# meyer-lab/cmtf-pls

Measured on AMD Instinct MI355X. Metric: nipals_iters_per_sec, higher is better.
Workload: dtype f32

## Files before the change

### cmtf_pls_amd/csrc/mixed.hip

```cpp
#include "common.hpp"

namespace cmtfpls {

typedef float f4_t __attribute__((ext_vector_type(4)));

#ifndef CMTFPLS_MIXED_UN
#define CMTFPLS_MIXED_UN 4
#endif
#ifndef CMTFPLS_MIXED_FAST
#define CMTFPLS_MIXED_FAST 1
#endif
#ifndef CMTFPLS_MIXED_UN_WIDE
#define CMTFPLS_MIXED_UN_WIDE 4
#endif

void launch_reduce_rows(const double* part, int nrows, int64_t P, double* out, hipStream_t st);

template <bool MASKED, bool VEC, int MT, bool FAST>
__global__ __launch_bounds__(256) void xcov_mixed_kernel(const float* __restrict__ X, int64_t I, int64_t P,
                                                        const double* __restrict__ Y, int ldy, int M,
                                                        double* __restrict__ part, int rows_per_block) {
  const int lane = threadIdx.x & 63, wv = threadIdx.x >> 6;
  const int kq = lane >> 4, nn = lane & 15;
  const int64_t cb = ((int64_t)blockIdx.x * 4 + wv) * 64;
  if (cb >= P) return;
  const int64_t c = cb + 4 * nn;
  const int64_t r0 = (int64_t)blockIdx.y * rows_per_block;
  const int64_t r1 = (r0 + rows_per_block < I) ? r0 + rows_per_block : I;
  using XV = Pack<float, 4>;
  f4_t acc32[MT][4];
  double acc64[MT][4][4];
#pragma unroll
  for (int mt = 0; mt < MT; ++mt)
#pragma unroll
    for (int e = 0; e < 4; ++e) {
      acc32[mt][e] = f4_t{0.f, 0.f, 0.f, 0.f};
#pragma unroll
      for (int g = 0; g < 4; ++g) acc64[mt][e][g] = 0.0;
    }
  bool mok[MT];
  int ycol[MT];
#pragma unroll
  for (int mt = 0; mt < MT; ++mt) { mok[mt] = (mt * 16 + nn) < M; ycol[mt] = mok[mt] ? mt * 16 + nn : M - 1; }
  constexpr int UN = (MT >= 2) ? CMTFPLS_MIXED_UN_WIDE : CMTFPLS_MIXED_UN;
  constexpr int FLUSH_TRIPS = 64 / (8 * UN);
  const int64_t cc = (c < P) ? c : (VEC ? P - 4 : P - 1);

  auto load_stage = [&](XV (&x)[UN], double (&a)[UN][MT], int64_t r) {
#pragma unroll
    for (int s = 0; s < UN; ++s) {
      const int64_t row = r + 4 * s + kq;
      const int64_t rowc = (FAST || row < r1) ? row : r1 - 1;
      if (VEC) {
        x[s] = ld_stream(reinterpret_cast<const XV*>(X + rowc * P + cc));
      } else {
#pragma unroll
        for (int e = 0; e < 4; ++e) x[s].e[e] = X[rowc * P + ((cc + e < P) ? cc + e : P - 1)];
      }
#pragma unroll
      for (int mt = 0; mt < MT; ++mt) a[s][mt] = Y[rowc * ldy + ycol[mt]];
    }
  };
  auto mma_stage = [&](const XV (&x)[UN], const double (&a)[UN][MT], int64_t r) {
#pragma unroll
    for (int s = 0; s < UN; ++s) {
      const bool rok = FAST || (r + 4 * s + kq) < r1;
      float af[MT];
#pragma unroll
      for (int mt = 0; mt < MT; ++mt) af[mt] = (FAST || (rok && mok[mt])) ? (float)a[s][mt] : 0.f;
#pragma unroll
      for (int e = 0; e < 4; ++e) {
        float xv = x[s].e[e];
        if (MASKED) xv = (xv == xv) ? xv : 0.f;
        const float b = (FAST || (rok && c + e < P)) ? xv : 0.f;
#pragma unroll
        for (int mt = 0; mt < MT; ++mt)
          acc32[mt][e] = __builtin_amdgcn_mfma_f32_16x16x4f32(af[mt], b, acc32[mt][e], 0, 0, 0);
      }
    }
  };
  auto flush = [&]() {
#pragma unroll
    for (int mt = 0; mt < MT; ++mt)
#pragma unroll
      for (int e = 0; e < 4; ++e) {
#pragma unroll
        for (int g = 0; g < 4; ++g) acc64[mt][e][g] += (double)acc32[mt][e][g];
        acc32[mt][e] = f4_t{0.f, 0.f, 0.f, 0.f};
      }
  };

  XV xa[UN], xb[UN];
  double aa[UN][MT], ab[UN][MT];
  load_stage(xa, aa, r0);
  int trip = 0;
  for (int64_t r = r0; r < r1; r += 8 * UN, ++trip) {
    load_stage(xb, ab, r + 4 * UN);
    __builtin_amdgcn_sched_barrier(0);
    mma_stage(xa, aa, r);
    __builtin_amdgcn_sched_barrier(0);
    load_stage(xa, aa, (FAST && r + 8 * UN >= r1) ? r : r + 8 * UN);
    __builtin_amdgcn_sched_barrier(0);
    mma_stage(xb, ab, r + 4 * UN);
    __builtin_amdgcn_sched_barrier(0);
    if (trip % FLUSH_TRIPS == FLUSH_TRIPS - 1) flush();
  }
  flush();
#pragma unroll
  for (int mt = 0; mt < MT; ++mt)
#pragma unroll
    for (int g = 0; g < 4; ++g) {
      const int m = mt * 16 + kq * 4 + g;
      if (m < M) {
        double* dst = part + ((int64_t)blockIdx.y * M + m) * P + c;
#pragma unroll
        for (int e = 0; e < 4; ++e)
          if (c + e < P) dst[e] = acc64[mt][e][g];
      }
    }
}

template <bool VEC, int RT>
__global__ __launch_bounds__(256) void mttkrp_mixed_kernel(const float* __restrict__ X, int64_t I, int A, int B,
                                                          const double* __restrict__ WA, const double* __restrict__ WB, int R,
                                                          double* __restrict__ out, int ldo) {
  extern __shared__ double lds[];
  constexpr int RP = 16 * RT;
  double* sA = lds;
  double* sB = lds + (size_t)A * RP;
  for (int idx = threadIdx.x; idx < A * RP; idx += 256) { const int j = idx / RP, r = idx % RP; sA[idx] = (r < R) ? WA[(int64_t)j * R + r] : 0.0; }
  for (int idx = threadIdx.x; idx < B * RP; idx += 256) { const int k = idx / RP, r = idx % RP; sB[idx] = (r < R) ? WB[(int64_t)k * R + r] : 0.0; }
  __syncthreads();
  const int lane = threadIdx.x & 63, wv = threadIdx.x >> 6;
  const int ri = lane & 15, kq = lane >> 4;
  const int64_t P = (int64_t)A * B;
  const int64_t ngroups = (I + 15) / 16;
  using XV = Pack<float, 4>;
  for (int64_t grp = (int64_t)blockIdx.x * 4 + wv; grp < ngroups; grp += (int64_t)gridDim.x * 4) {
    const int64_t i0 = grp * 16;
    const bool rok = (i0 + ri) < I;
    const float* __restrict__ xr = X + (rok ? i0 + ri : I - 1) * P;
    f4_t acc32[RT];
    double acc64[RT][4];
#pragma unroll
    for (int t = 0; t < RT; ++t) {
      acc32[t] = f4_t{0.f, 0.f, 0.f, 0.f};
#pragma unroll
      for (int g = 0; g < 4; ++g) acc64[t][g] = 0.0;
    }
    KronWalk w(4 * kq, 16, B);
    constexpr int UN = 4;
    int trip = 0;
    for (int64_t c0 = 0; c0 < P; c0 += 16 * UN, ++trip) {
      XV x[UN];
#pragma unroll
      for (int s = 0; s < UN; ++s) {
        const int64_t c = c0 + 16 * s + 4 * kq;
        if (VEC) {
          x[s] = ld_stream(reinterpret_cast<const XV*>(xr + ((c < P) ? c : P - 4)));
        } else {
#pragma unroll
          for (int e = 0; e < 4; ++e) x[s].e[e] = xr[(c + e < P) ? c + e : P - 1];
        }
      }
#pragma unroll
      for (int s = 0; s < UN; ++s) {
        const int64_t c = c0 + 16 * s + 4 * kq;
#pragma unroll
        for (int e = 0; e < 4; ++e) {
          const bool ok = rok && (c + e < P);
          const float a = ok ? x[s].e[e] : 0.f;
          int j = w.j, k = w.k + e;
          if (!VEC && k >= B) { j += k / B; k = k % B; }
          const bool wok = (c + e < P);
#pragma unroll
          for (int t = 0; t < RT; ++t) {
            const float b = wok ? (float)(sA[(size_t)j * RP + t * 16 + ri] * sB[(size_t)k * RP + t * 16 + ri]) : 0.f;
            acc32[t] = __builtin_amdgcn_mfma_f32_16x16x4f32(a, b, acc32[t], 0, 0, 0);
          }
        }
        w.next();
      }
      if ((trip & 3) == 3) {
#pragma unroll
        for (int t = 0; t < RT; ++t) {
#pragma unroll
          for (int g = 0; g < 4; ++g) acc64[t][g] += (double)acc32[t][g];
          acc32[t] = f4_t{0.f, 0.f, 0.f, 0.f};
        }
      }
    }
#pragma unroll
    for (int t = 0; t < RT; ++t)
#pragma unroll
      for (int g = 0; g < 4; ++g) {
        const int64_t row = i0 + kq * 4 + g;
        const int r = t * 16 + ri;
        if (row < I && r < R) out[row * ldo + r] = acc64[t][g] + (double)acc32[t][g];
      }
  }
}

template <int NL>
__global__ __launch_bounds__(256) void mttkrp_kj_mixed_kernel(const float* __restrict__ X, int64_t I, int A, int B,
                                                              const double* __restrict__ WA, const double* __restrict__ WB, int R,
                                                              double* __restrict__ out, int ldo) {
  constexpr int V = 4, RP = 16, CHJ = 8 / NL, KP = NL * 16 * V;
  constexpr int FLUSH = 64 / CHJ;
  extern __shared__ double lds[];
  double* sB = lds;
  float* sA = reinterpret_cast<float*>(lds + (size_t)B * RP);
  for (int idx = threadIdx.x; idx < A * RP; idx += 256) { const int j = idx / RP, r = idx % RP; sA[idx] = (r < R) ? (float)WA[(int64_t)j * R + r] : 0.f; }
  for (int idx = threadIdx.x; idx < B * RP; idx += 256) { const int k = idx / RP, r = idx % RP; sB[idx] = (r < R) ? WB[(int64_t)k * R + r] : 0.0; }
  __syncthreads();
  const int lane = threadIdx.x & 63, wv = threadIdx.x >> 6;
  const int kk = lane & 15, jq = lane >> 4;
  const int64_t P = (int64_t)A * B;
  const int npass = B / KP, cpp = A / (4 * CHJ);
  const int nchunks = npass * cpp, npairs = nchunks / 2;
  const int64_t istep = (int64_t)gridDim.x * 4;
  using XV = Pack<float, V>;
  XV b0[CHJ][NL], b1[CHJ][NL];
  auto load = [&](XV (&buf)[CHJ][NL], const float* __restrict__ xs, int q) {
    const int ps = q / cpp, c = q - ps * cpp;
    const float* __restrict__ xp = xs + (int64_t)(c * CHJ * 4) * B + ps * KP;
#pragma unroll
    for (int h = 0; h < CHJ; ++h)
#pragma unroll
      for (int n = 0; n < NL; ++n) buf[h][n] = ld_stream(reinterpret_cast<const XV*>(xp + (int64_t)(h * 4) * B + n * 16 * V));
  };
  int64_t i = (int64_t)blockIdx.x * 4 + wv;
  const int64_t lane_off = (int64_t)jq * B + V * kk;
  if (i < I) load(b0, X + i * P + lane_off, 0);
  for (; i < I; i += istep) {
    const float* __restrict__ xs = X + i * P + lane_off;
    const float* __restrict__ xs_next = X + ((i + istep < I) ? i + istep : i) * P + lane_off;
    double s = 0.0;
    f4_t acc[NL][V];
#pragma unroll
    for (int n = 0; n < NL; ++n)
#pragma unroll
      for (int e = 0; e < V; ++e) acc[n][e] = f4_t{0.f, 0.f, 0.f, 0.f};
    auto compute = [&](XV (&buf)[CHJ][NL], int q) {
      const int ps = q / cpp, c = q - ps * cpp;
      const float* __restrict__ sa = sA + (size_t)(c * CHJ * 4 + jq) * RP + kk;
#pragma unroll
      for (int h = 0; h < CHJ; ++h) {
        const float wa = sa[(size_t)(h * 4) * RP];
#pragma unroll
        for (int n = 0; n < NL; ++n)
#pragma unroll
          for (int e = 0; e < V; ++e) acc[n][e] = __builtin_amdgcn_mfma_f32_16x16x4f32(buf[h][n].e[e], wa, acc[n][e], 0, 0, 0);
      }
      if (c == cpp - 1 || (c % FLUSH) == FLUSH - 1) {
        const double* __restrict__ sb = sB + (size_t)(ps * KP) * RP + kk;
#pragma unroll
        for (int n = 0; n < NL; ++n)
#pragma unroll
          for (int e = 0; e < V; ++e) {
#pragma unroll
            for (int g = 0; g < 4; ++g) s = fma(sb[(size_t)(n * 16 * V + V * (4 * jq + g) + e) * RP], (double)acc[n][e][g], s);
            acc[n][e] = f4_t{0.f, 0.f, 0.f, 0.f};
          }
      }
    };
    for (int t = 0; t < npairs; ++t) {
      const int q = 2 * t;
      load(b1, xs, q + 1);
      compute(b0, q);
      const bool more = (q + 2 < nchunks);
      load(b0, more ? xs : xs_next, more ? q + 2 : 0);
      compute(b1, q + 1);
    }
    if (nchunks & 1) {
      compute(b0, nchunks - 1);
      load(b0, xs_next, 0);
    }
    s += __shfl_xor(s, 16, kWave);
    s += __shfl_xor(s, 32, kWave);
    if (jq == 0 && kk < R) out[i * ldo + kk] = s;
  }
}

}

using namespace cmtfpls;

extern "C" {

int cmtfpls_xcov_f32_mixed(const float* X, int64_t I, int64_t P, const double* Y, int ldy, int M, double* S, int masked,
                           void* ws, size_t ws_bytes, void* stream) {
  if (!X || !Y || !S || I <= 0 || P <= 0 || M <= 0 || ldy < M) { set_error("xcov_mixed: bad argument"); return CMTFPLS_EINVAL; }
  if (M > kXcovMaxResponses) {
    for (int lo = 0; lo < M; lo += kXcovMaxResponses) {
      const int mt = (M - lo < kXcovMaxResponses) ? M - lo : kXcovMaxResponses;
      const int rc = cmtfpls_xcov_f32_mixed(X, I, P, Y + lo, ldy, mt, S + (int64_t)lo * P, masked, ws, ws_bytes, stream);
      if (rc != CMTFPLS_OK) return rc;
    }
    return CMTFPLS_OK;
  }
  const XcovPlan p = plan_xcov(I, P);
  const size_t need = (size_t)p.row_blocks * M * P * sizeof(double);
  if (!ws || ws_bytes < need) { set_error("xcov_mixed: workspace too small"); return CMTFPLS_EWORKSPACE; }
  hipStream_t st = (hipStream_t)stream;
  const bool vec = (P % 4 == 0) && ((reinterpret_cast<uintptr_t>(X) & 15) == 0);
  const int mt = (M + 15) / 16;
  double* part = static_cast<double*>(ws);
  const dim3 grid(p.col_tiles, p.row_blocks), block(256);
  constexpr int kMaxUn = (CMTFPLS_MIXED_UN > CMTFPLS_MIXED_UN_WIDE) ? CMTFPLS_MIXED_UN : CMTFPLS_MIXED_UN_WIDE;
  const bool fast = CMTFPLS_MIXED_FAST && vec && (P % 256 == 0) && (M % 16 == 0) && (M / 16 != 3) && (I % p.rows_per_block == 0) &&
                    (p.rows_per_block % (8 * kMaxUn) == 0);
#define XL(MSK, VC, MTT, FS) hipLaunchKernelGGL((xcov_mixed_kernel<MSK, VC, MTT, FS>), grid, block, 0, st, X, I, P, Y, ldy, M, part, p.rows_per_block)
#define XM(MSK, VC, FS) do { if (mt == 1) XL(MSK, VC, 1, FS); else if (mt == 2) XL(MSK, VC, 2, FS); else XL(MSK, VC, 4, FS); } while (0)
  if (masked) { if (fast) XM(true, true, true); else if (vec) XM(true, true, false); else XM(true, false, false); }
  else        { if (fast) XM(false, true, true); else if (vec) XM(false, true, false); else XM(false, false, false); }
#undef XM
#undef XL
  launch_reduce_rows(part, p.row_blocks, (int64_t)M * P, S, st);
  return check_launch("xcov_mixed");
}

int cmtfpls_mttkrp_f32_mixed(const float* X, int64_t I, int A, int B, const double* WA, const double* WB, int R,
                             double* out, int ldo, void* stream) {
  if (!X || !WA || !WB || !out || I <= 0 || A <= 0 || B <= 0 || R <= 0 || ldo < R) { set_error("mttkrp_mixed: bad argument"); return CMTFPLS_EINVAL; }
  if (R > 32) { set_error("mttkrp_mixed: more than 32 components per call"); return CMTFPLS_EUNSUPPORTED; }
  const int rt = (R + 15) / 16;
  const size_t lds = (size_t)(A + B) * 16 * rt * sizeof(double);
  if (lds > 96 * 1024) { set_error("mttkrp_mixed: loadings exceed LDS"); return CMTFPLS_EUNSUPPORTED; }
  const bool vec = (B % 4 == 0) && ((reinterpret_cast<uintptr_t>(X) & 15) == 0);
  hipStream_t st = (hipStream_t)stream;
  if (R <= 16 && vec) {
    const size_t lds_kj = (size_t)B * 16 * sizeof(double) + (size_t)A * 16 * sizeof(float);
    int gk = (int)((I + 3) / 4);
    if (gk > 2048) gk = 2048;
    if (lds_kj <= 64 * 1024) {
      if (B % 128 == 0 && A % 16 == 0) {
        hipLaunchKernelGGL((mttkrp_kj_mixed_kernel<2>), dim3(gk), dim3(256), lds_kj, st, X, I, A, B, WA, WB, R, out, ldo);
        return check_launch("mttkrp_mixed");
      }
      if (B % 64 == 0 && A % 32 == 0) {
        hipLaunchKernelGGL((mttkrp_kj_mixed_kernel<1>), dim3(gk), dim3(256), lds_kj, st, X, I, A, B, WA, WB, R, out, ldo);
        return check_launch("mttkrp_mixed");
      }
    }
  }
  const int64_t ngroups = (I + 15) / 16;
  int grid = (int)((ngroups + 3) / 4);
  if (grid > 2048) grid = 2048;
#define ML(VC, RTT) hipLaunchKernelGGL((mttkrp_mixed_kernel<VC, RTT>), dim3(grid), dim3(256), lds, st, X, I, A, B, WA, WB, R, out, ldo)
  if (vec) { if (rt == 1) ML(true, 1); else ML(true, 2); }
  else     { if (rt == 1) ML(false, 1); else ML(false, 2); }
#undef ML
  return check_launch("mttkrp_mixed");
}

}
```

### cmtf_pls_amd/csrc/xcov.hip

```cpp
#include "common.hpp"

namespace cmtfpls {

typedef double d4_t __attribute__((ext_vector_type(4)));

void launch_reduce_rows(const double* part, int nrows, int64_t P, double* out, hipStream_t st);

XcovPlan plan_xcov(int64_t I, int64_t P) {
  XcovPlan p;
  p.col_tiles = (int)((P + 255) / 256);
#ifndef CMTFPLS_XCOV_BLOCKS
#define CMTFPLS_XCOV_BLOCKS 1024
#endif
  int64_t want = (CMTFPLS_XCOV_BLOCKS + p.col_tiles - 1) / p.col_tiles;
  if (want < 1) want = 1;
  int64_t rpb = (I + want - 1) / want;
  rpb = (rpb + 63) / 64 * 64;
  if (rpb < 64) rpb = 64;
  p.rows_per_block = (int)rpb;
  p.row_blocks = (int)((I + rpb - 1) / rpb);
  if (p.row_blocks < 1) p.row_blocks = 1;
  return p;
}

template <typename T, bool MASKED, bool VEC, int MT, bool FAST, bool SSQ = false, bool STATS = false>
__global__ __launch_bounds__(256) void xcov_kernel(const T* __restrict__ X, int64_t I, int64_t P,
                                                  const double* __restrict__ Y, int ldy, int M,
                                                  double* __restrict__ part, int rows_per_block,
                                                  const double* __restrict__ mean = nullptr, double* __restrict__ ssq_part = nullptr) {
  const int lane = threadIdx.x & 63, wv = threadIdx.x >> 6;
  const int kq = lane >> 4, nn = lane & 15;
  const int64_t cb = ((int64_t)blockIdx.x * 4 + wv) * 64;
  if (cb >= P) {
    if (SSQ && lane == 0) ssq_part[((int64_t)blockIdx.y * gridDim.x + blockIdx.x) * 4 + wv] = 0.0;
    return;
  }
  const int64_t c = cb + 4 * nn;
  const int64_t r0 = (int64_t)blockIdx.y * rows_per_block;
  const int64_t r1 = (r0 + rows_per_block < I) ? r0 + rows_per_block : I;
  using XV = Pack<T, 4>;
  d4_t acc[MT][4];
#pragma unroll
  for (int mt = 0; mt < MT; ++mt)
#pragma unroll
    for (int e = 0; e < 4; ++e) acc[mt][e] = d4_t{0.0, 0.0, 0.0, 0.0};
  bool mok[MT];
#pragma unroll
  for (int mt = 0; mt < MT; ++mt) mok[mt] = (mt * 16 + nn) < M;

#ifndef CMTFPLS_XCOV_UN
#define CMTFPLS_XCOV_UN 4
#endif
  constexpr int UN = CMTFPLS_XCOV_UN;
  const int64_t cc = (c < P) ? c : (VEC ? P - 4 : P - 1);
  int ycol[MT];
#pragma unroll
  for (int mt = 0; mt < MT; ++mt) ycol[mt] = mok[mt] ? mt * 16 + nn : M - 1;
  double mu[SSQ ? 4 : 1], ssq = 0.0;
  double cs[STATS ? 4 : 1] = {}, cq[STATS ? 4 : 1] = {};
  if constexpr (SSQ) {
#pragma unroll
    for (int e = 0; e < 4; ++e) mu[e] = mean[(c + e < P) ? c + e : P - 1];
  }

  auto load_stage = [&](XV (&x)[UN], double (&a)[UN][MT], int64_t r) {
#pragma unroll
    for (int s = 0; s < UN; ++s) {
      const int64_t row = r + 4 * s + kq;
      const int64_t rowc = (FAST || row < r1) ? row : r1 - 1;
      if (VEC) {
        x[s] = ld_stream(reinterpret_cast<const XV*>(X + rowc * P + cc));
      } else {
#pragma unroll
        for (int e = 0; e < 4; ++e) x[s].e[e] = X[rowc * P + ((cc + e < P) ? cc + e : P - 1)];
      }
#pragma unroll
      for (int mt = 0; mt < MT; ++mt) a[s][mt] = Y[rowc * ldy + ycol[mt]];
    }
  };
  auto mma_stage = [&](const XV (&x)[UN], const double (&a)[UN][MT], int64_t r) {
#pragma unroll
    for (int s = 0; s < UN; ++s) {
      const bool rok = FAST || (r + 4 * s + kq) < r1;
#pragma unroll
      for (int e = 0; e < 4; ++e) {
        const double xv = to_f64_masked<MASKED>(x[s].e[e]);
        const double b = (FAST || (rok && c + e < P)) ? xv : 0.0;
        if constexpr (SSQ) {
          const double dv = (FAST || (rok && c + e < P)) ? b - mu[e] : 0.0;
          ssq = fma(dv, dv, ssq);
        }
        if constexpr (STATS) {
          cs[e] += b;
          cq[e] = fma(b, b, cq[e]);
        }
#pragma unroll
        for (int mt = 0; mt < MT; ++mt)
          acc[mt][e] = __builtin_amdgcn_mfma_f64_16x16x4f64((FAST || (rok && mok[mt])) ? a[s][mt] : 0.0, b, acc[mt][e], 0, 0, 0);
      }
    }
  };

  XV xa[UN], xb[UN];
  double aa[UN][MT], ab[UN][MT];
  load_stage(xa, aa, r0);
  for (int64_t r = r0; r < r1; r += 8 * UN) {
    load_stage(xb, ab, r + 4 * UN);
    mma_stage(xa, aa, r);
    load_stage(xa, aa, (FAST && r + 8 * UN >= r1) ? r : r + 8 * UN);
    mma_stage(xb, ab, r + 4 * UN);
  }
  if constexpr (SSQ) {
    ssq = wave_sum(ssq);
    if (lane == 0) ssq_part[((int64_t)blockIdx.y * gridDim.x + blockIdx.x) * 4 + wv] = ssq;
  }
  if constexpr (STATS) {
    double* srow = ssq_part + (int64_t)blockIdx.y * 2 * P;
#pragma unroll
    for (int e = 0; e < 4; ++e) {
      double v = cs[e], w = cq[e];
      v += __shfl_xor(v, 16, kWave);
      v += __shfl_xor(v, 32, kWave);
      w += __shfl_xor(w, 16, kWave);
      w += __shfl_xor(w, 32, kWave);
      if (kq == 0 && c + e < P) { srow[c + e] = v; srow[P + c + e] = w; }
    }
  }
#pragma unroll
  for (int mt = 0; mt < MT; ++mt)
#pragma unroll
    for (int g = 0; g < 4; ++g) {
      const int m = mt * 16 + kq + 4 * g;
      if (m < M) {
        double* dst = part + ((int64_t)blockIdx.y * M + m) * P + c;
#pragma unroll
        for (int e = 0; e < 4; ++e)
          if (c + e < P) dst[e] = acc[mt][e][g];
      }
    }
}

template <typename T, int MT, bool FAST>
__global__ __launch_bounds__(256) void xcov_deflate_kernel(T* __restrict__ X, int64_t I, int64_t P, int B,
                                                          const double* __restrict__ Y, int ldy, int M,
                                                          double* __restrict__ part, int rows_per_block,
                                                          const double* __restrict__ t, const double* __restrict__ wA,
                                                          const double* __restrict__ wB, double* __restrict__ ssq_part) {
  const int lane = threadIdx.x & 63, wv = threadIdx.x >> 6;
  const int kq = lane >> 4, nn = lane & 15;
  const int64_t cb = ((int64_t)blockIdx.x * 4 + wv) * 64;
  if (cb >= P) {
    if (lane == 0) ssq_part[((int64_t)blockIdx.y * gridDim.x + blockIdx.x) * 4 + wv] = 0.0;
    return;
  }
  const int64_t c = cb + 4 * nn;
  const int64_t r0 = (int64_t)blockIdx.y * rows_per_block;
  const int64_t r1 = (r0 + rows_per_block < I) ? r0 + rows_per_block : I;
  using XV = Pack<T, 4>;
  d4_t acc[MT][4];
#pragma unroll
  for (int mt = 0; mt < MT; ++mt)
#pragma unroll
    for (int e = 0; e < 4; ++e) acc[mt][e] = d4_t{0.0, 0.0, 0.0, 0.0};
  bool mok[MT];
#pragma unroll
  for (int mt = 0; mt < MT; ++mt) mok[mt] = (mt * 16 + nn) < M;
  constexpr int UN = CMTFPLS_XCOV_UN;
  const bool cok = c < P;
  const int64_t cc = cok ? c : P - 4;
  int ycol[MT];
#pragma unroll
  for (int mt = 0; mt < MT; ++mt) ycol[mt] = mok[mt] ? mt * 16 + nn : M - 1;
  double wa[4], wb[4], ssq = 0.0;
#pragma unroll
  for (int e = 0; e < 4; ++e) {
    wa[e] = wA[(cc + e) / B];
    wb[e] = wB[(cc + e) % B];
  }

  auto load_stage = [&](XV (&x)[UN], double (&a)[UN][MT], double (&ts)[UN], int64_t r) {
#pragma unroll
    for (int s = 0; s < UN; ++s) {
      const int64_t row = r + 4 * s + kq;
      const int64_t rowc = (FAST || row < r1) ? row : r1 - 1;
      x[s] = ld_stream(reinterpret_cast<const XV*>(X + rowc * P + cc));
      ts[s] = t[rowc];
#pragma unroll
      for (int mt = 0; mt < MT; ++mt) a[s][mt] = Y[rowc * ldy + ycol[mt]];
    }
  };
  auto mma_stage = [&](XV (&x)[UN], const double (&a)[UN][MT], const double (&ts)[UN], int64_t r) {
#pragma unroll
    for (int s = 0; s < UN; ++s) {
      const int64_t row = r + 4 * s + kq;
      const bool rok = FAST || row < r1;
      const bool ok = rok && (FAST || cok);
#pragma unroll
      for (int e = 0; e < 4; ++e) {
        const double tw = ts[s] * wa[e];
        const T nv = (T)fma(-tw, wb[e], (double)x[s].e[e]);
        x[s].e[e] = nv;
        const double b = (ok && nv == nv) ? (double)nv : 0.0;
        ssq = fma(b, b, ssq);
#pragma unroll
        for (int mt = 0; mt < MT; ++mt)
          acc[mt][e] = __builtin_amdgcn_mfma_f64_16x16x4f64((FAST || (rok && mok[mt])) ? a[s][mt] : 0.0, b, acc[mt][e], 0, 0, 0);
      }
      if (ok) st_stream(reinterpret_cast<XV*>(X + row * P + c), x[s]);
    }
  };

  XV xa[UN], xb[UN];
  double aa[UN][MT], ab[UN][MT], ta[UN], tb[UN];
  load_stage(xa, aa, ta, r0);
  for (int64_t r = r0; r < r1; r += 8 * UN) {
    load_stage(xb, ab, tb, r + 4 * UN);
    mma_stage(xa, aa, ta, r);
    load_stage(xa, aa, ta, (r + 8 * UN >= r1) ? r : r + 8 * UN);
    mma_stage(xb, ab, tb, r + 4 * UN);
  }
  ssq = wave_sum(ssq);
  if (lane == 0) ssq_part[((int64_t)blockIdx.y * gridDim.x + blockIdx.x) * 4 + wv] = ssq;
#pragma unroll
  for (int mt = 0; mt < MT; ++mt)
#pragma unroll
    for (int g = 0; g < 4; ++g) {
      const int m = mt * 16 + kq + 4 * g;
      if (m < M) {
        double* dst = part + ((int64_t)blockIdx.y * M + m) * P + c;
#pragma unroll
        for (int e = 0; e < 4; ++e)
          if (c + e < P) dst[e] = acc[mt][e][g];
      }
    }
}

__global__ __launch_bounds__(256) void quadform_kernel(const double* __restrict__ G, int M, const double* __restrict__ q,
                                                      const double* __restrict__ q_old, double* __restrict__ out) {
  __shared__ double red[16];
  double s = 0.0;
  for (int idx = threadIdx.x; idx < M * M; idx += 256) {
    const int i = idx / M, j = idx - i * M;
    s = fma((q[i] - q_old[i]) * G[idx], (q[j] - q_old[j]), s);
  }
  s = block_sum(s, red);
  if (threadIdx.x == 0) out[0] = s;
}

static size_t xcov_ssq_extra(const XcovPlan& p) { return ((size_t)p.row_blocks * p.col_tiles * 4 * sizeof(double) + 255) / 256 * 256; }

template <typename T>
static int run_xcov_tile(const T* X, int64_t I, int64_t P, const double* Y, int ldy, int M, double* S, int masked,
                         void* ws, size_t ws_bytes, hipStream_t st, const double* mean = nullptr, double* ssq_out = nullptr,
                         double* stats_out = nullptr) {
  const XcovPlan p = plan_xcov(I, P);
  const bool with_ssq = ssq_out != nullptr, with_stats = stats_out != nullptr;
  if (with_ssq && (masked || !mean)) { set_error("xcov_ssq: needs the column means and a block without missing values"); return CMTFPLS_EINVAL; }
  if (with_stats && (masked || with_ssq)) { set_error("xcov_stats: a block without missing values, no second norm"); return CMTFPLS_EINVAL; }
  const size_t need = (size_t)p.row_blocks * M * P * sizeof(double) + (with_ssq ? xcov_ssq_extra(p) : 0) +
                      (with_stats ? (size_t)p.row_blocks * 2 * P * sizeof(double) : 0);
  if (!ws || ws_bytes < need) { set_error("xcov: workspace too small"); return CMTFPLS_EWORKSPACE; }
  const bool vec = (P % 4 == 0) && ((reinterpret_cast<uintptr_t>(X) & (4 * sizeof(T) - 1)) == 0);
  const int mt = (M + 15) / 16;
  double* part = static_cast<double*>(ws);
  const dim3 grid(p.col_tiles, p.row_blocks), block(256);
  const bool fast = vec && (P % 256 == 0) && (M % 16 == 0) && (M / 16 != 3) && (I % p.rows_per_block == 0) &&
                    (p.rows_per_block % (8 * 4) == 0);
  double* ssq_part = (with_ssq || with_stats) ? reinterpret_cast<double*>(static_cast<char*>(ws) + (size_t)p.row_blocks * M * P * sizeof(double)) : nullptr;
#define XL(MSK, VC, MTT, FS) hipLaunchKernelGGL((xcov_kernel<T, MSK, VC, MTT, FS>), grid, block, 0, st, X, I, P, Y, ldy, M, part, p.rows_per_block, (const double*)nullptr, (double*)nullptr)
#define XS(VC, MTT, FS) hipLaunchKernelGGL((xcov_kernel<T, false, VC, MTT, FS, true>), grid, block, 0, st, X, I, P, Y, ldy, M, part, p.rows_per_block, mean, ssq_part)
#define XM(MSK, VC, FS) do { if (mt == 1) XL(MSK, VC, 1, FS); else if (mt == 2) XL(MSK, VC, 2, FS); else XL(MSK, VC, 4, FS); } while (0)
#define XQ(VC, FS) do { if (mt == 1) XS(VC, 1, FS); else if (mt == 2) XS(VC, 2, FS); else XS(VC, 4, FS); } while (0)
#define XT1(VC, MTT, FS) hipLaunchKernelGGL((xcov_kernel<T, false, VC, MTT, FS, false, true>), grid, block, 0, st, X, I, P, Y, ldy, M, part, p.rows_per_block, (const double*)nullptr, ssq_part)
#define XT(VC, FS) do { if (mt == 1) XT1(VC, 1, FS); else if (mt == 2) XT1(VC, 2, FS); else XT1(VC, 4, FS); } while (0)
  if (with_stats)  { if (fast) XT(true, true); else if (vec) XT(true, false); else XT(false, false); }
  else if (with_ssq) {
    if constexpr (sizeof(T) == 2) { set_error("xcov_ssq: no 16-bit form; xcov_stats gives the norm"); return CMTFPLS_EUNSUPPORTED; }
    else { if (fast) XQ(true, true); else if (vec) XQ(true, false); else XQ(false, false); }
  }
  else if (masked) { if (fast) XM(true, true, true); else if (vec) XM(true, true, false); else XM(true, false, false); }
  else             { if (fast) XM(false, true, true); else if (vec) XM(false, true, false); else XM(false, false, false); }
#undef XT
#undef XT1
#undef XQ
#undef XM
#undef XS
#undef XL
  launch_reduce_rows(part, p.row_blocks, (int64_t)M * P, S, st);
  if (with_stats) launch_reduce_rows(ssq_part, p.row_blocks, 2 * P, stats_out, st);
  int rc = check_launch("xcov");
  if (rc == CMTFPLS_OK && with_ssq) rc = cmtfpls_sum_f64(ssq_part, (int64_t)p.row_blocks * p.col_tiles * 4, ssq_out, st);
  return rc;
}

template <typename T>
static int run_xcov(const T* X, int64_t I, int64_t P, const double* Y, int ldy, int M, double* S, int masked,
                    void* ws, size_t ws_bytes, hipStream_t st, const double* mean = nullptr, double* ssq_out = nullptr) {
  if (!X || !Y || !S || I <= 0 || P <= 0 || M <= 0 || ldy < M) { set_error("xcov: bad argument"); return CMTFPLS_EINVAL; }
  for (int lo = 0; lo < M; lo += kXcovMaxResponses) {
    const int mt = (M - lo < kXcovMaxResponses) ? M - lo : kXcovMaxResponses;
    const int rc = run_xcov_tile<T>(X, I, P, Y + lo, ldy, mt, S + (int64_t)lo * P, masked, ws, ws_bytes, st, mean, lo == 0 ? ssq_out : nullptr);
    if (rc != CMTFPLS_OK) return rc;
  }
  return CMTFPLS_OK;
}

template <typename T>
static int run_xcov_deflate(T* X, int64_t I, int A, int B, const double* Y, int ldy, int M, const double* t, const double* wA,
                            const double* wB, double* S, double* ssq, void* ws, size_t ws_bytes, hipStream_t st) {
  if (!X || !Y || !S || !t || !wA || !wB || !ssq || I <= 0 || A <= 0 || B <= 0 || M <= 0 || ldy < M) {
    set_error("xcov_deflate: bad argument");
    return CMTFPLS_EINVAL;
  }
  const int64_t P = (int64_t)A * B;
  if (M > 64 || (P % 4) != 0 || (reinterpret_cast<uintptr_t>(X) & (4 * sizeof(T) - 1)) != 0) {
    set_error("xcov_deflate: M > 64 or rows that are not whole 4-element vectors; deflate, then xcov");
    return CMTFPLS_EUNSUPPORTED;
  }
  const XcovPlan p = plan_xcov(I, P);
  const size_t need = (size_t)p.row_blocks * M * P * sizeof(double) + xcov_ssq_extra(p);
  if (!ws || ws_bytes < need) { set_error("xcov_deflate: workspace too small"); return CMTFPLS_EWORKSPACE; }
  const int mt = (M + 15) / 16;
  double* part = static_cast<double*>(ws);
  double* ssq_part = reinterpret_cast<double*>(static_cast<char*>(ws) + (size_t)p.row_blocks * M * P * sizeof(double));
  const dim3 grid(p.col_tiles, p.row_blocks), block(256);
  const bool fast = (P % 256 == 0) && (M % 16 == 0) && (M / 16 != 3) && (I % p.rows_per_block == 0) && (p.rows_per_block % (8 * 4) == 0);
#define XD(MTT, FS) hipLaunchKernelGGL((xcov_deflate_kernel<T, MTT, FS>), grid, block, 0, st, X, I, P, B, Y, ldy, M, part, p.rows_per_block, t, wA, wB, ssq_part)
  if (fast) { if (mt == 1) XD(1, true); else if (mt == 2) XD(2, true); else XD(4, true); }
  else      { if (mt == 1) XD(1, false); else if (mt == 2) XD(2, false); else XD(4, false); }
#undef XD
  launch_reduce_rows(part, p.row_blocks, (int64_t)M * P, S, st);
  int rc = check_launch("xcov_deflate");
  if (rc == CMTFPLS_OK) rc = cmtfpls_sum_f64(ssq_part, (int64_t)p.row_blocks * p.col_tiles * 4, ssq, st);
  return rc;
}

}

using namespace cmtfpls;

extern "C" {

size_t cmtfpls_xcov_workspace_bytes(int64_t I, int64_t P, int M) {
  if (I <= 0 || P <= 0 || M <= 0) return 0;
  const XcovPlan p = plan_xcov(I, P);
  if (M > kXcovMaxResponses) M = kXcovMaxResponses;
  return (size_t)p.row_blocks * M * P * sizeof(double);
}
int cmtfpls_xcov_f32(const float* X, int64_t I, int64_t P, const double* Y, int ldy, int M, double* S, int masked,
                     void* ws, size_t ws_bytes, void* stream) {
  return run_xcov<float>(X, I, P, Y, ldy, M, S, masked, ws, ws_bytes, (hipStream_t)stream);
}
int cmtfpls_xcov_f64(const double* X, int64_t I, int64_t P, const double* Y, int ldy, int M, double* S, int masked,
                     void* ws, size_t ws_bytes, void* stream) {
  return run_xcov<double>(X, I, P, Y, ldy, M, S, masked, ws, ws_bytes, (hipStream_t)stream);
}
int cmtfpls_xcov_bf16(const uint16_t* X, int64_t I, int64_t P, const double* Y, int ldy, int M, double* S, int masked,
                      void* ws, size_t ws_bytes, void* stream) {
  return run_xcov<bf16_t>(reinterpret_cast<const bf16_t*>(X), I, P, Y, ldy, M, S, masked, ws, ws_bytes, (hipStream_t)stream);
}
int cmtfpls_xcov_f16(const uint16_t* X, int64_t I, int64_t P, const double* Y, int ldy, int M, double* S, int masked,
                     void* ws, size_t ws_bytes, void* stream) {
  return run_xcov<f16_t>(reinterpret_cast<const f16_t*>(X), I, P, Y, ldy, M, S, masked, ws, ws_bytes, (hipStream_t)stream);
}
size_t cmtfpls_xcov_ssq_workspace_bytes(int64_t I, int64_t P, int M) {
  if (I <= 0 || P <= 0 || M <= 0) return 0;
  const XcovPlan p = plan_xcov(I, P);
  if (M > kXcovMaxResponses) M = kXcovMaxResponses;
  return (size_t)p.row_blocks * M * P * sizeof(double) + xcov_ssq_extra(p);
}
int cmtfpls_xcov_ssq_f32(const float* X, int64_t I, int64_t P, const double* Y, int ldy, int M, double* S, const double* mean,
                         double* ssq, void* ws, size_t ws_bytes, void* stream) {
  if (!mean || !ssq) { set_error("xcov_ssq: bad argument"); return CMTFPLS_EINVAL; }
  return run_xcov<float>(X, I, P, Y, ldy, M, S, 0, ws, ws_bytes, (hipStream_t)stream, mean, ssq);
}
int cmtfpls_xcov_ssq_f64(const double* X, int64_t I, int64_t P, const double* Y, int ldy, int M, double* S, const double* mean,
                         double* ssq, void* ws, size_t ws_bytes, void* stream) {
  if (!mean || !ssq) { set_error("xcov_ssq: bad argument"); return CMTFPLS_EINVAL; }
  return run_xcov<double>(X, I, P, Y, ldy, M, S, 0, ws, ws_bytes, (hipStream_t)stream, mean, ssq);
}
size_t cmtfpls_xcov_stats_workspace_bytes(int64_t I, int64_t P, int M) {
  if (I <= 0 || P <= 0 || M <= 0 || M > kXcovMaxResponses) return 0;
  const XcovPlan p = plan_xcov(I, P);
  return (size_t)p.row_blocks * ((size_t)M + 2) * P * sizeof(double);
}
int cmtfpls_xcov_stats_f32(const float* X, int64_t I, int64_t P, const double* Y, int ldy, int M, double* S, double* stats,
                           void* ws, size_t ws_bytes, void* stream) {
  if (!X || !Y || !S || !stats || I <= 0 || P <= 0 || M <= 0 || ldy < M) { set_error("xcov_stats: bad argument"); return CMTFPLS_EINVAL; }
  if (M > kXcovMaxResponses) { set_error("xcov_stats: more than 64 responses; use colstats + xcov"); return CMTFPLS_EUNSUPPORTED; }
  return run_xcov_tile<float>(X, I, P, Y, ldy, M, S, 0, ws, ws_bytes, (hipStream_t)stream, nullptr, nullptr, stats);
}
int cmtfpls_xcov_stats_f64(const double* X, int64_t I, int64_t P, const double* Y, int ldy, int M, double* S, double* stats,
                           void* ws, size_t ws_bytes, void* stream) {
  if (!X || !Y || !S || !stats || I <= 0 || P <= 0 || M <= 0 || ldy < M) { set_error("xcov_stats: bad argument"); return CMTFPLS_EINVAL; }
  if (M > kXcovMaxResponses) { set_error("xcov_stats: more than 64 responses; use colstats + xcov"); return CMTFPLS_EUNSUPPORTED; }
  return run_xcov_tile<double>(X, I, P, Y, ldy, M, S, 0, ws, ws_bytes, (hipStream_t)stream, nullptr, nullptr, stats);
}
int cmtfpls_xcov_stats_bf16(const uint16_t* X, int64_t I, int64_t P, const double* Y, int ldy, int M, double* S, double* stats,
                            void* ws, size_t ws_bytes, void* stream) {
  if (!X || !Y || !S || !stats || I <= 0 || P <= 0 || M <= 0 || ldy < M) { set_error("xcov_stats: bad argument"); return CMTFPLS_EINVAL; }
  if (M > kXcovMaxResponses) { set_error("xcov_stats: more than 64 responses; use xcov"); return CMTFPLS_EUNSUPPORTED; }
  return run_xcov_tile<bf16_t>(reinterpret_cast<const bf16_t*>(X), I, P, Y, ldy, M, S, 0, ws, ws_bytes, (hipStream_t)stream, nullptr, nullptr, stats);
}
int cmtfpls_xcov_stats_f16(const uint16_t* X, int64_t I, int64_t P, const double* Y, int ldy, int M, double* S, double* stats,
                           void* ws, size_t ws_bytes, void* stream) {
  if (!X || !Y || !S || !stats || I <= 0 || P <= 0 || M <= 0 || ldy < M) { set_error("xcov_stats: bad argument"); return CMTFPLS_EINVAL; }
  if (M > kXcovMaxResponses) { set_error("xcov_stats: more than 64 responses; use xcov"); return CMTFPLS_EUNSUPPORTED; }
  return run_xcov_tile<f16_t>(reinterpret_cast<const f16_t*>(X), I, P, Y, ldy, M, S, 0, ws, ws_bytes, (hipStream_t)stream, nullptr, nullptr, stats);
}
int cmtfpls_xcov_deflate_f32(float* X, int64_t I, int A, int B, const double* Y, int ldy, int M, const double* t, const double* wA,
                             const double* wB, double* S, double* ssq, void* ws, size_t ws_bytes, void* stream) {
  return run_xcov_deflate<float>(X, I, A, B, Y, ldy, M, t, wA, wB, S, ssq, ws, ws_bytes, (hipStream_t)stream);
}
int cmtfpls_xcov_deflate_f64(double* X, int64_t I, int A, int B, const double* Y, int ldy, int M, const double* t, const double* wA,
                             const double* wB, double* S, double* ssq, void* ws, size_t ws_bytes, void* stream) {
  return run_xcov_deflate<double>(X, I, A, B, Y, ldy, M, t, wA, wB, S, ssq, ws, ws_bytes, (hipStream_t)stream);
}
int cmtfpls_quadform_f64(const double* G, int M, const double* q, const double* q_old, double* out, void* stream) {
  if (!G || !q || !q_old || !out || M <= 0) { set_error("quadform: bad argument"); return CMTFPLS_EINVAL; }
  hipLaunchKernelGGL(quadform_kernel, dim3(1), dim3(256), 0, (hipStream_t)stream, G, M, q, q_old, out);
  return check_launch("quadform");
}

}
```

Baseline: 765.7.

## Tune xcov waves-per-EU, precompute 32-bit lane offsets, pin load/compute schedule

Adds amdgpu_waves_per_eu attributes to the xcov, mixed xcov and deflate kernels, chosen per tile width, so the compiler can trade register use for occupancy. In the fast path, loads now take a uniform row base plus a precomputed 32-bit per-lane byte offset instead of per-lane 64-bit row arithmetic. Scheduling barriers are placed between the load and MMA stages of the double-buffered loop. The fast path is gated on the offsets fitting in 32 bits. The occupancy hints may force register spills, and the barriers may block useful interleaving by the compiler.

```diff
diff --git a/cmtf_pls_amd/csrc/mixed.hip b/cmtf_pls_amd/csrc/mixed.hip
--- a/cmtf_pls_amd/csrc/mixed.hip
+++ b/cmtf_pls_amd/csrc/mixed.hip
@@ -1,4 +1,5 @@
 #include "common.hpp"
+#include "xcov_waves.hpp"
 
 namespace cmtfpls {
 
@@ -17,7 +18,8 @@
 void launch_reduce_rows(const double* part, int nrows, int64_t P, double* out, hipStream_t st);
 
 template <bool MASKED, bool VEC, int MT, bool FAST>
-__global__ __launch_bounds__(256) void xcov_mixed_kernel(const float* __restrict__ X, int64_t I, int64_t P,
+__global__ __launch_bounds__(256) CMTFPLS_XCOV_WAVES(MT, VEC)
+void xcov_mixed_kernel(const float* __restrict__ X, int64_t I, int64_t P,
                                                         const double* __restrict__ Y, int ldy, int M,
                                                         double* __restrict__ part, int rows_per_block) {
   const int lane = threadIdx.x & 63, wv = threadIdx.x >> 6;
@@ -46,9 +48,20 @@
   constexpr int FLUSH_TRIPS = 64 / (8 * UN);
   const int64_t cc = (c < P) ? c : (VEC ? P - 4 : P - 1);
 
+  const uint32_t xoff = (uint32_t)((kq * P + cc) * (int64_t)sizeof(float));
+  const uint32_t yoff = (uint32_t)(((int64_t)kq * ldy + nn) * (int64_t)sizeof(double));
+
   auto load_stage = [&](XV (&x)[UN], double (&a)[UN][MT], int64_t r) {
 #pragma unroll
     for (int s = 0; s < UN; ++s) {
+      if constexpr (FAST) {
+        const char* xr = reinterpret_cast<const char*>(X + (r + 4 * s) * P);
+        const char* yr = reinterpret_cast<const char*>(Y + (r + 4 * s) * ldy);
+        x[s] = ld_stream(reinterpret_cast<const XV*>(xr + xoff));
+#pragma unroll
+        for (int mt = 0; mt < MT; ++mt) a[s][mt] = *reinterpret_cast<const double*>(yr + yoff + mt * 16 * sizeof(double));
+        continue;
+      }
       const int64_t row = r + 4 * s + kq;
       const int64_t rowc = (FAST || row < r1) ? row : r1 - 1;
       if (VEC) {
@@ -309,7 +322,7 @@
   const dim3 grid(p.col_tiles, p.row_blocks), block(256);
   constexpr int kMaxUn = (CMTFPLS_MIXED_UN > CMTFPLS_MIXED_UN_WIDE) ? CMTFPLS_MIXED_UN : CMTFPLS_MIXED_UN_WIDE;
   const bool fast = CMTFPLS_MIXED_FAST && vec && (P % 256 == 0) && (M % 16 == 0) && (M / 16 != 3) && (I % p.rows_per_block == 0) &&
-                    (p.rows_per_block % (8 * kMaxUn) == 0);
+                    (p.rows_per_block % (8 * kMaxUn) == 0) && xcov_lane_offsets_fit(P, sizeof(float), ldy);
 #define XL(MSK, VC, MTT, FS) hipLaunchKernelGGL((xcov_mixed_kernel<MSK, VC, MTT, FS>), grid, block, 0, st, X, I, P, Y, ldy, M, part, p.rows_per_block)
 #define XM(MSK, VC, FS) do { if (mt == 1) XL(MSK, VC, 1, FS); else if (mt == 2) XL(MSK, VC, 2, FS); else XL(MSK, VC, 4, FS); } while (0)
   if (masked) { if (fast) XM(true, true, true); else if (vec) XM(true, true, false); else XM(true, false, false); }
diff --git a/cmtf_pls_amd/csrc/xcov.hip b/cmtf_pls_amd/csrc/xcov.hip
--- a/cmtf_pls_amd/csrc/xcov.hip
+++ b/cmtf_pls_amd/csrc/xcov.hip
@@ -1,4 +1,5 @@
 #include "common.hpp"
+#include "xcov_waves.hpp"
 
 namespace cmtfpls {
 
@@ -23,8 +24,16 @@
   return p;
 }
 
+template <typename T, bool VEC, bool FAST, bool SSQ, bool STATS>
+constexpr bool xcov_four() {
+  if (sizeof(T) == 8) return false;
+  if (FAST) return true;
+  return !STATS && !(SSQ && !VEC);
+}
+
 template <typename T, bool MASKED, bool VEC, int MT, bool FAST, bool SSQ = false, bool STATS = false>
-__global__ __launch_bounds__(256) void xcov_kernel(const T* __restrict__ X, int64_t I, int64_t P,
+__global__ __launch_bounds__(256) CMTFPLS_XCOV_WAVES(MT, (xcov_four<T, VEC, FAST, SSQ, STATS>()))
+void xcov_kernel(const T* __restrict__ X, int64_t I, int64_t P,
                                                   const double* __restrict__ Y, int ldy, int M,
                                                   double* __restrict__ part, int rows_per_block,
                                                   const double* __restrict__ mean = nullptr, double* __restrict__ ssq_part = nullptr) {
@@ -63,9 +72,20 @@
     for (int e = 0; e < 4; ++e) mu[e] = mean[(c + e < P) ? c + e : P - 1];
   }
 
+  const uint32_t xoff = (uint32_t)((kq * P + cc) * (int64_t)sizeof(T));
+  const uint32_t yoff = (uint32_t)(((int64_t)kq * ldy + nn) * (int64_t)sizeof(double));
+
   auto load_stage = [&](XV (&x)[UN], double (&a)[UN][MT], int64_t r) {
 #pragma unroll
     for (int s = 0; s < UN; ++s) {
+      if constexpr (FAST) {
+        const char* xr = reinterpret_cast<const char*>(X + (r + 4 * s) * P);
+        const char* yr = reinterpret_cast<const char*>(Y + (r + 4 * s) * ldy);
+        x[s] = ld_stream(reinterpret_cast<const XV*>(xr + xoff));
+#pragma unroll
+        for (int mt = 0; mt < MT; ++mt) a[s][mt] = *reinterpret_cast<const double*>(yr + yoff + mt * 16 * sizeof(double));
+        continue;
+      }
       const int64_t row = r + 4 * s + kq;
       const int64_t rowc = (FAST || row < r1) ? row : r1 - 1;
       if (VEC) {
@@ -104,11 +124,16 @@
   XV xa[UN], xb[UN];
   double aa[UN][MT], ab[UN][MT];
   load_stage(xa, aa, r0);
+  auto pin = [] { if constexpr (FAST) __builtin_amdgcn_sched_barrier(0); };
   for (int64_t r = r0; r < r1; r += 8 * UN) {
     load_stage(xb, ab, r + 4 * UN);
+    pin();
     mma_stage(xa, aa, r);
+    pin();
     load_stage(xa, aa, (FAST && r + 8 * UN >= r1) ? r : r + 8 * UN);
+    pin();
     mma_stage(xb, ab, r + 4 * UN);
+    pin();
   }
   if constexpr (SSQ) {
     ssq = wave_sum(ssq);
@@ -141,7 +166,8 @@
 }
 
 template <typename T, int MT, bool FAST>
-__global__ __launch_bounds__(256) void xcov_deflate_kernel(T* __restrict__ X, int64_t I, int64_t P, int B,
+__global__ __launch_bounds__(256) __attribute__((amdgpu_waves_per_eu(MT == 1 ? 2 : 1, 2)))
+void xcov_deflate_kernel(T* __restrict__ X, int64_t I, int64_t P, int B,
                                                           const double* __restrict__ Y, int ldy, int M,
                                                           double* __restrict__ part, int rows_per_block,
                                                           const double* __restrict__ t, const double* __restrict__ wA,
@@ -265,7 +291,7 @@
   double* part = static_cast<double*>(ws);
   const dim3 grid(p.col_tiles, p.row_blocks), block(256);
   const bool fast = vec && (P % 256 == 0) && (M % 16 == 0) && (M / 16 != 3) && (I % p.rows_per_block == 0) &&
-                    (p.rows_per_block % (8 * 4) == 0);
+                    (p.rows_per_block % (8 * 4) == 0) && xcov_lane_offsets_fit(P, sizeof(T), ldy);
   double* ssq_part = (with_ssq || with_stats) ? reinterpret_cast<double*>(static_cast<char*>(ws) + (size_t)p.row_blocks * M * P * sizeof(double)) : nullptr;
 #define XL(MSK, VC, MTT, FS) hipLaunchKernelGGL((xcov_kernel<T, MSK, VC, MTT, FS>), grid, block, 0, st, X, I, P, Y, ldy, M, part, p.rows_per_block, (const double*)nullptr, (double*)nullptr)
 #define XS(VC, MTT, FS) hipLaunchKernelGGL((xcov_kernel<T, false, VC, MTT, FS, true>), grid, block, 0, st, X, I, P, Y, ldy, M, part, p.rows_per_block, mean, ssq_part)
diff --git a/cmtf_pls_amd/csrc/xcov_waves.hpp b/cmtf_pls_amd/csrc/xcov_waves.hpp
--- /dev/null
+++ b/cmtf_pls_amd/csrc/xcov_waves.hpp
@@ -0,0 +1,15 @@
+#pragma once
+#include <stddef.h>
+#include <stdint.h>
+
+namespace cmtfpls {
+
+constexpr int xcov_waves_min(int mt, bool four) { return mt == 1 ? (four ? 4 : 2) : (mt == 2 ? 2 : 1); }
+constexpr int xcov_waves_max(int mt, bool four) { return (mt == 1 && four) ? 8 : 2; }
+#define CMTFPLS_XCOV_WAVES(MT, FOUR) __attribute__((amdgpu_waves_per_eu(cmtfpls::xcov_waves_min(MT, FOUR), cmtfpls::xcov_waves_max(MT, FOUR))))
+
+inline bool xcov_lane_offsets_fit(int64_t P, size_t elem, int ldy) {
+  return 4 * (uint64_t)P * elem < (1ull << 32) && 4 * (uint64_t)ldy * sizeof(double) < (1ull << 32);
+}
+
+}
```

New measurement: 765.9, median of 2. No clear change (+0.0%).
